# GadGadGad/Convolutional-KAN-for-Image-Classification

Hardware: AMD Instinct MI355X
Metric: images/sec fwd+bwd KAN-VGG11 3x32x32 bs=256/GPU (higher is better)
Workload: dtype f32

## Files before the change

### convolutional-kan-for-image-classification_amd/_lib.py

```python
from __future__ import annotations

import ctypes as C
import os
from typing import Optional

_HERE = os.path.dirname(os.path.abspath(__file__))
LIB_PATH = os.environ.get("KANCONV_LIB") or os.path.join(_HERE, "libkanconv.so")

KAN_MAX_PLANES = 16
KAN_MAX_TABLE = 32
KAN_FP_WORDS = 192
BASIS_BSPLINE, BASIS_RBF, BASIS_CHEBY, BASIS_POLY, BASIS_FOURIER, BASIS_RELU, BASIS_GRAM = 0, 1, 2, 3, 4, 5, 6
ACT_NONE, ACT_IDENTITY, ACT_GELU, ACT_SILU, ACT_RELU, ACT_TANH, ACT_SIGMOID, ACT_GELU_TANH = -1, 0, 1, 2, 3, 4, 5, 6
ORDER_QUAD_FWD, ORDER_ROWBLK8_FWD, ORDER_QUAD_BWD_DATA, ORDER_FWD_WEIGHT_SIDE = 1, 2, 4, 8


class KanGeom(C.Structure):
    _fields_ = [(n, C.c_int) for n in ("B", "C", "H", "W", "O", "Ho", "Wo", "kh", "kw", "sh", "sw", "ph", "pw", "dh", "dw", "groups")] + \
               [("x_bstride", C.c_longlong), ("y_bstride", C.c_longlong)]


class KanBasis(C.Structure):
    _fields_ = [("kind", C.c_int), ("n_basis", C.c_int), ("order", C.c_int), ("act", C.c_int),
                ("p0", C.c_float), ("p1", C.c_float), ("table", C.c_float * KAN_MAX_TABLE), ("chan_table", C.c_void_p)]


class KanPlan(C.Structure):
    _fields_ = [(n, C.c_int) for n in ("P", "K", "IPC", "KC", "Kpad", "Opad", "fwd_splits", "bwd_data_splits", "bwd_weight_splits",
                                          "fwd_target", "bwd_data_target", "bwd_weight_target", "x_pm_wanted", "dz_pm_wanted", "bwd_weight_expanded", "row_blocks", "e_pm_wanted", "fwd_expanded", "fwd_halo", "bwd_weight_halo",
                                          "fwd_band", "bwd_weight_band")] + \
               [(n, C.c_longlong) for n in ("packed_weight_bytes", "bwd_data_weight_bytes", "fwd_slab_elems", "bwd_data_slab_elems",
                                            "bwd_weight_slab_elems", "e_pm_elems")]


class KanNormRoute(C.Structure):
    _fields_ = [(n, C.c_int) for n in ("kernel", "G", "EPL", "PPI", "NT", "pool", "lds", "held", "blocks", "strided")]

# ... 127 lines not shown
```

### convolutional-kan-for-image-classification_amd/csrc/kan_internal.h

```cpp
#pragma once
#include <type_traits>
#include "kanconv.h"

int kan_fail_msg(const char* fmt, const char* a);
int kan_raise_lds_limit(const void* kernel, int bytes);

enum : int {
    FAST_GENERIC = 0,
    FAST_BSPLINE_SILU = 1,
    FAST_BSPLINE_GELU = 2,
    FAST_RBF8 = 3,
    FAST_CHEBY5 = 4,
    FAST_CHEBY4 = 5,
    FAST_POLY4 = 6,
    FAST_POLY3 = 7,
    FAST_RBF5 = 8,
    FAST_RELU8 = 9,
    FAST_GRAM4 = 10,
    FAST_POLY1 = 11,
    FAST_LAST = 11
};
enum : unsigned {
    ON_TAP_MAJOR = 1u << 0,
    ON_BIG_TILES = 1u << 1,
// ... 84 lines not shown
int kan_band_bwd_weight_launch(const float* dz, const float* x, const float* xn, float* dwp, const KanGeom* g, const KanBasis* b,
                               const KanBandCfg* cfg, int splits, long long slab_elems, void* stream);
int kan_band_fwd_launch(const float* x, const float* xn, const float* wp, float* z, const KanGeom* g, const KanBasis* b,
                        const KanBandCfg* cfg, int splits, long long slab_elems, void* stream);

constexpr int DW_T = 9;
constexpr int DW_MAX_TP = 96;

enum class Route { TAP_MAJOR, DW, BAND, HALO, EXPANDED };

struct FwdCfg { int TO, TP, tiles_o, tiles_p, chunks, splits, slots; };
struct BdCfg { int CH, tiles_c, tiles_p, n_ob, Opad32, chunks, splits; };
struct BwCfg { int TR, TO, tiles_r, tiles_o, chunks, splits, slots; };
struct BwHaloCfg { int R, nimg, spb, n_bands, tiles_r, tiles_o, splits, bands_per_split; };

struct ConvPlan {
    KanPlan pub;
    int fast;
    Route fwd, bwd_data, bwd_weight;
    bool pm_fwd, pm_bwd_data, pm_bwd_weight;
    bool rowblk_bwd_data;
    bool quad_fwd;
    bool quad_bd;
    bool rowblk8_fwd;
    bool fwd_wq;
    bool pmdma_xcd, pm_lpt, pm_xcd;
    FwdCfg fc;
    BdCfg bd;
    BwCfg bw;
    BwHaloCfg bwh;
    KanBandCfg band;
};
int plan_conv(const KanGeom* g, const KanBasis* b, ConvPlan* cp);

int live_taps_out(const KanGeom* g, int hw);
int live_taps_in(const KanGeom* g, int hw);
int live_positions_for_tap(const KanGeom* g, int tap);
int balance_tiles(const int* weight, int n, unsigned short* idx);
```

### convolutional-kan-for-image-classification_amd/csrc/kan_plan.hip

```cpp
#include <hip/hip_runtime.h>
#include <cstdio>
#include <cstdlib>
#include <cstring>
#include "kanconv.h"
#include "kan_device.h"
#include "kan_common.h"
#include "kan_internal.h"

namespace {

int fail(const char* msg) { return kan_fail_msg("%s", msg); }

int check(const KanGeom* g, const KanBasis* b) {
    if (!g || !b) return fail("null geometry/basis");
    if (g->groups < 0 || g->groups > 65535) return fail("groups out of range");
    if (g->B <= 0 || g->C <= 0 || g->O <= 0 || g->H <= 0 || g->W <= 0 || g->Ho <= 0 || g->Wo <= 0) return fail("non-positive dimension");
    if (g->kh <= 0 || g->kw <= 0 || g->sh <= 0 || g->sw <= 0 || g->dh <= 0 || g->dw <= 0 || g->ph < 0 || g->pw < 0) return fail("bad conv parameters");
    if (g->kh > 255 || g->kw > 255 || g->C > 65535) return fail("kernel size / channel count out of supported range");
    if ((g->H + 2 * g->ph - g->dh * (g->kh - 1) - 1) / g->sh + 1 != g->Ho || (g->W + 2 * g->pw - g->dw * (g->kw - 1) - 1) / g->sw + 1 != g->Wo)
        return fail("Ho/Wo inconsistent with H/W, kernel, stride, padding, dilation");
    if ((long long)g->B * g->Ho * g->Wo >= (1ll << 31) || (long long)g->B * g->H * g->W >= (1ll << 31)) return fail("pixel count exceeds int32");
    if ((long long)g->B * g->x_bstride * 4 >= (1ll << 31) || (long long)g->B * g->y_bstride * 4 >= (1ll << 31))
        return fail("activation tensors must be smaller than 2 GiB (32-bit buffer offsets)");
    if (g->x_bstride < (long long)ngroups(g) * g->C * g->H * g->W || g->y_bstride < (long long)ngroups(g) * g->O * g->Ho * g->Wo)
// ... 318 lines not shown
    pl->Opad = round_up(g->O, 64);
    pl->packed_weight_bytes = (long long)G * pl->Kpad * pl->Opad * 4;
    c.bd = bd_cfg(g, *pl);
    pl->bwd_data_weight_bytes = (long long)G * T * c.bd.Opad32 * c.bd.tiles_c * 128 * 4;
    pl->fwd_slab_elems = (long long)g->B * g->y_bstride;
    pl->bwd_data_slab_elems = (long long)g->B * g->x_bstride;
    pl->bwd_weight_slab_elems = (long long)G * pl->K * pl->Opad;
    const bool big = big_tiles(f, *pl);
    c.fc = fwd_cfg(g, *pl, big, c.pm_fwd, halo);
    c.bw = bw_cfg(g, *pl, big, c.pm_bwd_weight);
    if (halo_bw) c.bwh = bw_halo_cfg(g, *pl);
    pl->fwd_splits = band ? c.band.fwd_splits : c.fc.splits;
    pl->bwd_data_splits = c.bd.splits;
    pl->bwd_weight_splits = halo_bw ? c.bwh.splits : c.bw.splits;
    if (band_bw) {
        pl->bwd_weight_splits = c.band.bw_splits;
        pl->bwd_weight_slab_elems = (long long)G * pl->Kpad * pl->Opad;
    }
    pl->fwd_target = pl->bwd_data_target = pl->bwd_weight_target = 0;
    const bool rowblk_fwd = halo && g->H == 4 && g->W == 4 && c.fc.TO == 256;
    c.quad_fwd = rowblk_fwd && g->B % 32 == 0 && !tuning_off("KAN_QUAD_FWD");
    c.quad_bd = c.rowblk_bwd_data && g->B % 32 == 0 && !tuning_off("KAN_QUAD_BD");
    c.rowblk8_fwd = halo && g->H == 8 && g->W == 8 && c.fc.TO == 256 && g->B % 4 == 0 && !tuning_off("KAN_ROWBLK8_FWD");
    c.fwd_wq = c.fwd == Route::EXPANDED && g->H == 2 && g->W == 2 && g->Ho == 2 && g->Wo == 2 && g->kh == 3 && g->kw == 3 && g->sh == 1 && g->sw == 1 &&
               g->ph == 1 && g->pw == 1 && g->dh == 1 && g->dw == 1 && pl->P == 9 && pl->KC == 18 && g->y_bstride % 4 == 0 && !tuning_off("KAN_PMDMA_FWD_WQ");
    if (dw) {
        pl->fwd_splits = pl->bwd_data_splits = 1;
        pl->bwd_weight_splits = dw_weight_chunks(g);
        pl->bwd_data_weight_bytes = pl->packed_weight_bytes;
        c.pm_fwd = c.pm_bwd_data = c.pm_bwd_weight = false;
    }
    if (c.pm_fwd) {
        LiveClass cls[16]; const int plane = g->Ho * g->Wo;
        const long long tiles_per_pos = (long long)ceil_div(g->B, c.fc.TP) * c.fc.tiles_o * G;
        for (int hw = 0; hw < plane; ++hw) cls[hw] = LiveClass{tiles_per_pos, live_taps_out(g, hw) * ceil_div(g->C, pl->IPC)};
        pl->fwd_target = pick_target_steps(cls, plane, 8, 4.0 * g->B * g->O * g->Ho * g->Wo * G, &pl->fwd_splits, c.fc.slots);
    }
    if (c.pm_bwd_weight) {
        LiveClass cw[32];
        const long long tiles_per_tap = (long long)ceil_div((long long)g->C * pl->P, c.bw.TR) * c.bw.tiles_o * G;
        for (int tap = 0; tap < T; ++tap) cw[tap] = LiveClass{tiles_per_tap, live_positions_for_tap(g, tap) * ceil_div(g->B, 16)};
        pl->bwd_weight_target = pick_target_steps(cw, T, 16, 4.0 * pl->K * pl->Opad * G, &pl->bwd_weight_splits, c.bw.slots);
    }
    if (c.pm_bwd_data) {
        LiveClass cls[16]; const int plane = g->H * g->W;
        const long long tiles_per_pos = (long long)ceil_div(g->B, 128) * c.bd.tiles_c * G;
// ... 17 lines not shown
```

### convolutional-kan-for-image-classification_amd/csrc/kanconv.hip

```cpp
#include <hip/hip_runtime.h>
#include <cstdio>
#include <cstdlib>
#include <cstring>
#include <cmath>
#include <cstdint>
#include <mutex>
#include <type_traits>
#include <vector>
#include "kanconv.h"
#include "kan_device.h"

#include "kan_common.h"
#include "kan_internal.h"

namespace {


thread_local char g_err[512] = "";
int fail(const char* fmt, const char* a = "") {
    snprintf(g_err, sizeof(g_err), fmt, a);
    return -1;
}
}
int kan_fail_msg(const char* fmt, const char* a) { return fail(fmt, a); }
// ... 741 lines not shown
    do {                                                                                                                           \
        float fa_[2][2], fb_[2][2];                                                                                                \
        LDS_READ4(fa_[0][0], fa_[0][1], fb_[0][0], fb_[0][1], addrA, addrB, 0, 32 * 4, 0, 512 * 4);                                \
        _Pragma("unroll") for (int kk = 0; kk < (NK); ++kk) {                                                                       \
            const int c_ = kk & 1, n_ = c_ ^ 1;                                                                                    \
            if (kk + 1 < (NK)) {                                                                                                   \
                LDS_READ4(fa_[n_][0], fa_[n_][1], fb_[n_][0], fb_[n_][1], addrA, addrB, (2 * (kk + 1)) * (LDA) * 4,                \
                          (2 * (kk + 1)) * (LDA) * 4 + 128, (2 * (kk + 1)) * 32 * 4, (2 * (kk + 1)) * 32 * 4 + 512 * 4);           \
                LDS_WAIT4(fa_[c_][0], fa_[c_][1], fb_[c_][0], fb_[c_][1], 4);                                                      \
            } else {                                                                                                               \
                LDS_WAIT4(fa_[c_][0], fa_[c_][1], fb_[c_][0], fb_[c_][1], 0);                                                      \
            }                                                                                                                      \
            if (l0) {                                                                                                              \
                acc[0][0] = MFMA32(fa_[c_][0], fb_[c_][0], acc[0][0]);                                                             \
                acc[1][0] = MFMA32(fa_[c_][1], fb_[c_][0], acc[1][0]);                                                             \
            }                                                                                                                      \
            if (l1) {                                                                                                              \
                acc[0][1] = MFMA32(fa_[c_][0], fb_[c_][1], acc[0][1]);                                                             \
                acc[1][1] = MFMA32(fa_[c_][1], fb_[c_][1], acc[1][1]);                                                             \
            }                                                                                                                      \
        }                                                                                                                          \
    } while (0)

template <int KIND, int FAST, int RB = 0>
__global__ __launch_bounds__(256, 4) void k_conv_bwd_data(
    const float* __restrict__ dz, const float* __restrict__ x, const float* __restrict__ xn, const float* __restrict__ wd,
    float* __restrict__ dx, float* __restrict__ dxn, DevGeom g, DevBasis bs, int CH, int n_ct, int n_ob, int Opad16,
    int n_chunks, int chunks_per_split, long long slab_elems, unsigned dz_bytes, TilePerm perm, float* __restrict__ dpar) {
    constexpr int TP = 128, KD = 16, NT = 256;
    __shared__ __attribute__((aligned(16))) float smem[2 * 2 * KD * 128];
    __shared__ float sTab[KAN_MAX_TABLE];

    const int tid = threadIdx.x, lane = tid & 63;
    const int wave = __builtin_amdgcn_readfirstlane(tid >> 6);
    const int w_r = wave >> 1, w_p = wave & 1;
    const int HoWo = g.Ho * g.Wo, HW = g.H * g.W, P = bs.P;
    const int Min = g.B * HW;
    const BlockId blk = xcd_block_order(false);
    const int grp = blk.y / n_ct;
    const int px_tile0 = (perm.n ? (int)perm.idx[blk.x] : blk.x) * TP, ct = blk.y - grp * n_ct;
    const int ncol = n_ct * 128;
    const int pxl = (wave & 1) * 64 + lane, ol0 = wave >> 1;
    const bool idle_rows = (ct * 2 + w_r) * CH >= g.C;
    {
        const size_t xo = (size_t)grp * g.C * HW;
        x += xo; xn += xo; dx += xo; if (dxn) dxn += xo;
        dz += (size_t)grp * g.O * HoWo * ((g.pix_major || RB == 2) ? g.B : 1);
        wd += (size_t)grp * (g.kh * g.kw) * Opad16 * ncol;
    }

    if (tid < KAN_MAX_TABLE) sTab[tid] = bs.tab[tid];
    const int q_qh = (blk.x >> 1) & 1, q_qw = blk.x & 1, q_b0 = (blk.x >> 2) * 32;
    auto q_pos = [&](int bk) { return ((bk == 0 || bk == 2) ? 3 * q_qh : 1 + q_qh) * 4 + ((bk == 0 || bk == 3) ? 3 * q_qw : 1 + q_qw); };
    auto q_mask = [&](int hw) {
        unsigned m = 0;
        for (int tap = 0; tap < 9; ++tap) {
            const int r = tap / 3, t = tap - r * 3;
            m |= (((unsigned)((hw >> 2) + 1 - r) < 4u && (unsigned)((hw & 3) + 1 - t) < 4u) ? 1u : 0u) << tap;
        }
        return m;
    };
    const int my_px = RB == 2 ? (q_b0 + (pxl & 31)) * 16 + q_pos(pxl >> 5)
                              : px_tile0 + (RB == 1 ? ((pxl >> 2) & 7) * 16 + (pxl >> 5) * 4 + (pxl & 3) : pxl);
    const bool pv = my_px < Min;
    int pb, ph_, pw_;
    {
        int hw;
        if (g.pix_major) { hw = my_px / g.B; pb = my_px - hw * g.B; }
        else { pb = my_px / HW; hw = my_px - pb * HW; }
        ph_ = hw / g.W; pw_ = hw - ph_ * g.W;
// ... 89 lines not shown
    const unsigned q_live0 = q_mask(q_pos(2 * w_p)), q_live1 = q_mask(q_pos(2 * w_p + 1));
    const unsigned q_voff = (unsigned)((lane >> 3) * 16 * g.B + (lane & 7) * 4) * 4u;
    int pend_tap = 0;
    auto issue_q = [&](int ch, int buf) {
        const int tap = ch / n_ob, o0 = (ch - tap * n_ob) * KD;
        pend_tap = tap;
        float* dW = smem + buf * (2 * KD * 128);
        float* dG = dW + KD * 128 + wv * 512;
        if ((cp_live >> tap) & 1u) {
            const int r = tap / 3, t = tap - r * 3;
            const unsigned so = (unsigned)((o0 * 16 + cp_hw + (1 - r) * 4 + (1 - t)) * g.B + q_b0) * 4u;
            __builtin_amdgcn_raw_ptr_buffer_load_lds(dz_rs, (__attribute__((address_space(3))) void*)dG, 16, (int)q_voff, (int)so, 0, 0);
            __builtin_amdgcn_raw_ptr_buffer_load_lds(dz_rs, (__attribute__((address_space(3))) void*)(dG + 256), 16, (int)q_voff,
                                                     (int)(so + (unsigned)(8 * 16 * g.B) * 4u), 0, 0);
        }
        const char* wsrc = (const char*)(wd + ((size_t)tap * Opad16 + o0) * ncol + ct * 128);
#pragma unroll
        for (int j = 0; j < 2; ++j) {
            const int blk2 = j * 4 + wv;
            glds16((const float*)(wsrc + (size_t)blk2 * 2 * ncol * 4 + wlane), dW + blk2 * 256);
        }
    };

    f32x16 acc[2][2];
#pragma unroll
    for (int a = 0; a < 2; ++a)
#pragma unroll
        for (int b = 0; b < 2; ++b)
#pragma unroll
            for (int r = 0; r < 16; ++r) acc[a][b][r] = 0.f;

    int ch0 = blk.z * chunks_per_split;
    int ch1 = min(n_chunks, ch0 + chunks_per_split);
    unsigned tapmask = 0xffffffffu;
    if (g.pix_major) {
        tapmask = 0;
        const int T = g.kh * g.kw;
        const int hwA = px_tile0 / g.B, hwB = min(px_tile0 + TP - 1, Min - 1) / g.B;
        for (int hw = hwA; hw <= hwB; ++hw)
            for (int tap = 0; tap < T; ++tap) tapmask |= (tap_alive_in(g, hw, tap) ? 1u : 0u) << tap;
        auto seg = [&](int tap) { return tap * n_ob; };
        const int L = live_step_count(tapmask, T, n_chunks, seg);
        const int S = min((int)gridDim.z, max(1, (L + chunks_per_split - 1) / chunks_per_split));
        if (blk.z >= S) { ch0 = ch1 = n_chunks; }
        else {
            ch0 = blk.z == 0 ? 0 : live_step_pos(tapmask, T, n_chunks, (int)((long long)L * blk.z / S), seg);
            ch1 = blk.z == S - 1 ? n_chunks : live_step_pos(tapmask, T, n_chunks, (int)((long long)L * (blk.z + 1) / S), seg);
        }
    }
    auto next_live = [&](int ch) -> int {
        if (!g.pix_major) return ch;
        while (ch < ch1) {
            const int tap = ch / n_ob;
            if ((tapmask >> tap) & 1u) return ch;
            ch = (tap + 1) * n_ob;
        }
        return ch1;
    };
    int ch = next_live(ch0);
    if (ch < ch1) { if (RB == 2) issue_q(ch, 0); else if (RB) issue_rb(ch, 0); else issue(ch, 0); }
    const int ar = w_r * 64 + (lane & 31), bp = w_p * 64 + (lane & 31), kh2 = lane >> 5;
    for (int cur = 0; ch < ch1; cur ^= 1) {
        asm volatile("s_waitcnt vmcnt(0)" ::: "memory");
        __syncthreads();
        const bool mixed_now = pend_mixed;
        const int tap_now = pend_tap;
        ch = next_live(ch + 1);
        if (ch < ch1) { if (RB == 2) issue_q(ch, cur ^ 1); else if (RB) issue_rb(ch, cur ^ 1); else issue(ch, cur ^ 1); }
        const float* cW = smem + cur * (2 * KD * 128);
        const float* cG = cW + KD * 128;
        const unsigned aw = lds_addr(cW + kh2 * 128 + ar), ag = lds_addr(cG + kh2 * TP + bp);
        if (RB == 2) {
            const unsigned agq = lds_addr(cG + (2 * w_p) * 512 + kh2 * 32 + (lane & 31));
            const bool l0 = ((q_live0 >> tap_now) & 1u) != 0, l1 = ((q_live1 >> tap_now) & 1u) != 0;
            if (!idle_rows) KAN_MFMA_STEP_QUAD(KD / 2, aw, 128, agq, l0, l1);
        } else if (RB) {
            const bool l0b = !(mixed_now && w_p == 0), l1a = !(mixed_now && w_p == 1);
            if (!idle_rows) KAN_MFMA_STEP_LIVE(KD / 2, aw, 128, ag, TP, true, l0b, l1a, true);
        } else if (!idle_rows) KAN_MFMA_STEP(KD / 2, aw, 128, ag, TP);
    }

    const bool same_in = (x == xn);
    const bool split_out = (dxn != nullptr);
    float* dxs = dx + (size_t)blk.z * slab_elems;
    float* dxns = split_out ? dxn + (size_t)blk.z * slab_elems : nullptr;
#define KAN_G_TO_LDS(half)                                                                                                 \
    __syncthreads();                                                                                                       \
    if (w_r == (half)) {                                                                                                   \
        _Pragma("unroll") for (int mi = 0; mi < 2; ++mi)                                                                   \
            _Pragma("unroll") for (int ni = 0; ni < 2; ++ni)                                                               \
                _Pragma("unroll") for (int r = 0; r < 16; ++r)                                                             \
                    smem[(mi * 32 + mfma_row(r, lane)) * TP + w_p * 64 + ni * 32 + (lane & 31)] = acc[mi][ni][r];          \
    }                                                                                                                      \
    __syncthreads();
    if constexpr (FAST != 0) {
        constexpr FastSpec S = fast_spec(FAST);
        constexpr int FP = S.planes, FCH = 64 / FP, NIT = (FCH + 1) / 2, NPF = S.xn_bwd ? 1 : 2;
        float xv[NPF][NIT], nv[NIT]; unsigned ok = 0;
#define KAN_FETCH(half, slot)                                                                                              \
        _Pragma("unroll") for (int it = 0; it < NIT; ++it) {                                                                   \
            const int cl = ol0 + 2 * it, c = (ct * 2 + (half)) * FCH + cl;                                                     \
            const bool v = cl < FCH && c < g.C && pv;                                                                          \
            const size_t idx = (size_t)pb * g.xbs + (size_t)c * HW + (size_t)(ph_ * g.W + pw_);                                \
            xv[slot][it] = v ? x[idx] : 0.f;                                                                                   \
            if constexpr (S.xn_bwd) nv[it] = v ? xn[idx] : 0.f;                                                                \
            ok |= (v ? 1u : 0u) << ((slot) * NIT + it);                                                                        \
        }
        if constexpr (!S.xn_bwd) {
#pragma unroll
            for (int half = 0; half < 2; ++half) KAN_FETCH(half, half)
        }
#pragma unroll 1
        for (int half = 0; half < 2; ++half) {
            if constexpr (S.xn_bwd) { ok = 0; KAN_FETCH(half, 0) }
            KAN_G_TO_LDS(half)
#pragma unroll
            for (int it = 0; it < NIT; ++it) {
                if (!((ok >> ((S.xn_bwd ? 0 : half) * NIT + it)) & 1u)) continue;
                const int cl = ol0 + 2 * it, c = (ct * 2 + half) * FCH + cl;
                const float xa = (S.xn_bwd || half == 0) ? xv[0][it] : xv[NPF - 1][it];
// ... 1721 lines not shown
        const int bx = c.tiles_c * 4, by = c.Opad32 / 32 * G;
        const long long nt = (long long)bx * by;
        const long long capd = fp ? 128 : 1024;
        dim3 gd((unsigned)(nt < capd ? nt : capd), 1, T);
        hipLaunchKernelGGL(k_pack_bwd_data, gd, dim3(256), 0, st, (const float*)wp, wd, q, c.CH, c.tiles_c, c.Opad32, wp_gs, bx, by, fp, fp_cur);
    }
    return launch_ok("pack");
}

int kan_pack_weights(const float* w_base, const float* w_basis, float* wp, float* wd, const KanGeom* g, const KanBasis* b, void* stream) {
    return pack_weights_impl(w_base, w_basis, wp, wd, g, b, nullptr, 0, stream);
}

int kan_pack_weights_iod(const float* coeffs, float* wp, float* wd, const KanGeom* g, const KanBasis* b, void* stream) {
    if (int rc = iod_scope(g, b)) return rc;
    return pack_weights_impl(nullptr, coeffs, wp, wd, g, b, nullptr, 0, stream, true);
}

int kan_tile_orders(const KanGeom* g, const KanBasis* b) {
    ConvPlan cp;
    if (plan_conv(g, b, &cp)) return 0;
    const bool halo = cp.fwd == Route::HALO;
    return (halo && cp.quad_fwd ? KAN_ORDER_QUAD_FWD : 0) | (halo && cp.rowblk8_fwd ? KAN_ORDER_ROWBLK8_FWD : 0) | (cp.quad_bd ? KAN_ORDER_QUAD_BWD_DATA : 0) |
           (cp.fwd_wq ? KAN_ORDER_FWD_WEIGHT_SIDE : 0);
}

int kan_pack_cacheable(const KanGeom* g, const KanBasis* b) {
    ConvPlan cp;
    if (plan_conv(g, b, &cp)) return 0;
    if ((long long)g->O * g->C * (b->n_basis + 1) * g->kh * g->kw >= (1ll << 31)) return 0;
    return (!pack_needs_clear(g, cp.pub) && cp.fwd != Route::DW && ngroups(g) == 1) ? 1 : 0;
}

int kan_pack_weights_cached(const float* w_base, const float* w_basis, float* wp, float* wd, const KanGeom* g, const KanBasis* b,
                            unsigned long long* ring, int cur, int force, int sample_stride, void* stream) {
    static_assert(KAN_FP_WORDS == 3 * FP_LANES, "ring size");
    if (!ring || cur < 0 || cur > 2 || sample_stride < 1) return fail("bad fingerprint ring arguments");
    if (!kan_pack_cacheable(g, b)) return fail("cached packing is not offered for this geometry (kan_pack_cacheable)");
    const int hb = b->act != KAN_ACT_NONE;
    if ((hb && !w_base) || !w_basis) return fail("null weight pointer");
    if (((size_t)w_basis & 15) || (hb && ((size_t)w_base & 15))) return fail("cached packing needs 16-byte aligned weight tensors");
    const int T = g->kh * g->kw;
    const long long na = hb ? (long long)g->O * g->C * T : 0, nbs = (long long)g->O * g->C * b->n_basis * T;
    const long long groups4 = ((na + 3) / 4 + (nbs + 3) / 4 + sample_stride - 1) / sample_stride;
    long long blocks = (groups4 + 256 * 8 - 1) / (256 * 8); if (blocks > 4096) blocks = 4096; if (blocks < 1) blocks = 1;
    hipLaunchKernelGGL(k_fingerprint, dim3((unsigned)blocks), dim3(256), 0, (hipStream_t)stream, hb ? w_base : w_basis, (unsigned)na, w_basis,
                       (unsigned)nbs, (unsigned)sample_stride, ring, cur);
// ... 166 lines not shown
        DevGeom dgd = dev_geom(g); DevBasis dbd = dev_basis(b);
        dim3 grid(ceil_div((long long)g->B * g->H * g->W, 256), ngroups(g));
        dispatch_kind(b->kind, [&](auto kind) {
            hipLaunchKernelGGL((k_dw_bwd_data<decltype(kind)::value>), grid, dim3(256), 0, st, dz, x, xn, wd, dx, dxn, dgd, dbd, pl.Opad, pl.IPC, pl.KC, pl.Kpad);
        });
        return launch_ok("dw_bwd_data");
    }
    const BdCfg& c = cp.bd;
    DevGeom dg = dev_geom(g);
    dg.pix_major = (dz_pm && cp.pm_bwd_data) ? 1 : 0;
    if (dg.pix_major) dz = dz_pm;
    DevBasis db = dev_basis(b);
    if ((long long)c.tiles_c * ngroups(g) > 65535) return fail("groups * channel tiles exceed the grid limit");
    dim3 grid(c.tiles_p, c.tiles_c * ngroups(g), pl.bwd_data_splits);
    const int cps = dg.pix_major ? pl.bwd_data_target : ceil_div(c.chunks, pl.bwd_data_splits);
    TilePerm perm; perm.n = 0;
    if (dg.pix_major) perm = tile_perm(c.tiles_p, [&](int t) {
        const int hw = (int)(((long long)t * 128) / g->B);
        return ceil_div(live_taps_in(g, hw < g->H * g->W ? hw : 0) * c.n_ob, cps > 0 ? cps : 1);
    });
    const int fast = (fast_spec(cp.fast).xn_bwd ? (x != xn && dxn) : (x == xn && !dxn)) ? cp.fast : FAST_GENERIC;
    const bool rb = !dg.pix_major && cp.rowblk_bwd_data;
    const bool quad = rb && cp.quad_bd && dz_pm && x == xn && !dxn;
    const unsigned dz_bytes = (unsigned)((long long)g->B * g->y_bstride * 4);
    auto launch = [&](auto kind, auto fast, auto rbv) {
        hipLaunchKernelGGL((k_conv_bwd_data<decltype(kind)::value, decltype(fast)::value, decltype(rbv)::value>), grid, dim3(256), 0, st,
                           decltype(rbv)::value == 2 ? dz_pm : dz, x, xn, wd,
                           dx, dxn, dg, db, c.CH, c.tiles_c, c.n_ob, c.Opad32, c.chunks, cps, pl.bwd_data_slab_elems, dz_bytes, perm, dpar);
    };
    const bool launched = dispatch_fast<ON_TAP_MAJOR>(fast, [&](auto fv) {
        constexpr int F = decltype(fv)::value;
        if constexpr (fast_has(F, ON_ROWBLK_BWD_DATA)) {
            if (quad) return launch(IC<fast_kind(F)>{}, fv, IC<2>{});
            if (rb) return launch(IC<fast_kind(F)>{}, fv, IC<1>{});
        }
        launch(IC<fast_kind(F)>{}, fv, IC<0>{});
    });
    if (!launched) dispatch_kind(b->kind, [&](auto kind) { launch(kind, IC<FAST_GENERIC>{}, IC<0>{}); });
    return launch_ok("conv_bwd_data");
}

int kan_conv_bwd_weight(const float* dz, const float* x, const float* xn, float* dwp, const KanGeom* g, const KanBasis* b,
                        const float* x_pm, const float* dz_pm, void* stream) {
    ConvPlan cp;
    if (int rc = plan_conv(g, b, &cp)) return rc;
    const KanPlan& pl = cp.pub;
    if (!dz || !x || !xn || !dwp) return fail("null tensor pointer");
    if ((b->kind == KAN_BASIS_RELU || b->kind == KAN_BASIS_GRAM) && !b->chan_table) return fail("ReLU / Gram bases need their device parameter table (chan_table)");
    hipStream_t st = (hipStream_t)stream;
    if (cp.bwd_weight == Route::DW) {
        DevGeom dgd = dev_geom(g); DevBasis dbd = dev_basis(b);
        dim3 grid(pl.bwd_weight_splits, ngroups(g));
        dispatch_kind(b->kind, [&](auto kind) {
            hipLaunchKernelGGL((k_dw_bwd_weight<decltype(kind)::value>), grid, dim3(256), 0, st, dz, x, xn, dwp, dgd, dbd, pl.K, pl.Opad, pl.bwd_weight_slab_elems);
        });
// ... 381 lines not shown
```

### convolutional-kan-for-image-classification_amd/ops.py

```python
from __future__ import annotations

import contextlib
import ctypes as C
import os
import weakref
from collections import OrderedDict
from dataclasses import dataclass, replace
from functools import lru_cache, partial, wraps
from typing import List, NamedTuple, Optional, Sequence, Tuple

import torch
from torch.autograd.function import once_differentiable

from . import _lib as L


@dataclass(frozen=True)
class ConvSpec:
    kind: int
    n_basis: int
    order: int
    act: int
    p0: float
    p1: float
# ... 157 lines not shown
        for wo in range(Wo):
            for r in range(kh):
                for t in range(kw):
                    hi, wi = ho * sh - ph + r * dh, wo * sw - pw + t * dw
                    live += 0 <= hi < H and 0 <= wi < W
    return live / float(Ho * Wo * kh * kw)


_ROW_BLOCK_BIT = {"fwd": 1, "bwd_data": 2, "bwd_weight": 0}


def _quadrant_order(geom, plan, which: str) -> bool:
    return which == "fwd" and bool(plan.row_blocks & 1) and geom.B % 32 == 0


def _quadrant_bwd_data(geom, plan, have_dz_pm: bool) -> bool:
    return bool(have_dz_pm) and bool(plan.row_blocks & 2) and bool(getattr(plan, "tile_orders", 0) & L.ORDER_QUAD_BWD_DATA)


def _row_blocks8_forward(geom, plan) -> bool:
    return geom.H == 8 and geom.W == 8 and bool(getattr(plan, "tile_orders", 0) & L.ORDER_ROWBLK8_FWD)


def _executed_flops(geom, plan, which: str, have_dz_pm: bool = False) -> float:
    target = {"fwd": plan.fwd_target, "bwd_data": plan.bwd_data_target, "bwd_weight": plan.bwd_weight_target}[which]
    dense = _conv_flops(geom, plan)
    g = geom
    if target <= 0:
        if _quadrant_order(geom, plan, which) or (which == "bwd_data" and _quadrant_bwd_data(geom, plan, have_dz_pm)):
            return dense * _live_fraction(which, g.H, g.W, g.Ho, g.Wo, g.kh, g.kw, g.sh, g.sw, g.ph, g.pw, g.dh, g.dw)
        if plan.row_blocks & _ROW_BLOCK_BIT[which]:
            return dense * (5.0 / 6.0)
        if which == "fwd" and _row_blocks8_forward(geom, plan):
            return dense * (11.0 / 12.0)
        return dense
    return dense * _live_fraction(which, g.H, g.W, g.Ho, g.Wo, g.kh, g.kw, g.sh, g.sw, g.ph, g.pw, g.dh, g.dw)


def _layer_tag(geom) -> str:
    return f"{geom.C * max(1, geom.groups)}->{geom.O * max(1, geom.groups)}@{geom.H}x{geom.W} k{geom.kh}x{geom.kw}"


def _sample(which: str, geom, plan, pm: bool, two: bool = False, expanded: bool = False):
    tile = "128" if plan.Opad % 128 == 0 else "64"
    if which == "bwd_data":
        name = "k_conv_bwd_data"
    elif expanded:
        name = f"k_conv_{which}_pmdma/o{tile}"
    elif plan.fwd_band if which == "fwd" else plan.bwd_weight_band:
        name = f"k_band_{which}/o" + ("128" if plan.Opad % 128 == 0 else "192" if plan.Opad == 192 else "64")
    else:
        halo = plan.fwd_halo if which == "fwd" else (plan.bwd_weight_halo and not two)
        name = f"k_conv_{which}{'_halo' if halo else ''}/o{tile}"
    skips = expanded or pm or bool(plan.row_blocks & _ROW_BLOCK_BIT[which]) or (which == "fwd" and _row_blocks8_forward(geom, plan))
    dense = _conv_flops(geom, plan)
    return name, dense, _executed_flops(geom, plan, which, pm) if skips else dense, _layer_tag(geom)

# ... 379 lines not shown
    ent.used = True
    return t


def _conv_backward(spec: ConvSpec, x, xn, packed, dz, need_x: bool, need_xn: bool, need_w: bool, phases=None, mode: int = 0, wids=None, dparams=None, wcd=None, dw_split: bool = False):
    lib = L.load()
    B, Ct, H, W = x.shape
    G = spec.groups
    Cg = Ct // G
    Ot = dz.shape[1]
    Og = Ot // G
    geom, basis, plan = _plan_cached(*_plan_key(spec, x.shape, Og))
    basis = _with_table(_with_phases(basis, phases, mode), spec, x.device)
    kh, kw = spec.kernel
    st = _stream(x)
    xs = xn if xn is not None else x
    wd, x_pm = packed
    dw_base: List[Optional[torch.Tensor]] = [None] * G
    dw_basis: List[Optional[torch.Tensor]] = [None] * G
    split_w = need_w and dw_split
    split_x = need_x and wcd is not None
    exact_w = need_w and not split_w
    exact_x = (need_x or need_xn) and not split_x
    dz_pm = _position_major(dz, 0, Ot) if (plan.dz_pm_wanted and xn is None and (exact_w or exact_x)) else None
    if split_w:
        sb, ss = (_sink_for(wids[0], (Og, Cg, kh, kw), x.device), _sink_for(wids[1], (Og, Cg * spec.n_basis, kh, kw), x.device)) if wids else (None, None)
        dwb = sb if sb is not None else torch.empty((Og, Cg, kh, kw), device=x.device, dtype=torch.float32)
        dws = ss if ss is not None else torch.empty((Og, Cg * spec.n_basis, kh, kw), device=x.device, dtype=torch.float32)
        kan_conv_bwd_weight_split(spec, x, dz, out=(dwb, dws))
        dw_base, dw_basis = list(dwb.unsqueeze(0).unbind(0)), list(dws.unsqueeze(0).unbind(0))
    elif exact_w:
        dwp = torch.empty(plan.bwd_weight_splits * plan.bwd_weight_slab_elems, device=x.device, dtype=torch.float32)
        if plan.bwd_weight_expanded and xn is None and dz_pm is not None:
            e_pm = x_pm if (plan.fwd_expanded and not plan.x_pm_wanted and x_pm is not None and mode == 0) else _expand_pm(x, geom, basis, plan, st)
            _launch(_sample("bwd_weight", geom, plan, True, expanded=True), x,
                    lambda: lib.kan_conv_bwd_weight_expanded(_ptr(dz_pm), _ptr(e_pm), _ptr(dwp), C.byref(geom), C.byref(basis), st))
        else:
            _launch(_sample("bwd_weight", geom, plan, x_pm is not None and dz_pm is not None, xn is not None), x,
                    lambda: lib.kan_conv_bwd_weight(_ptr(dz), _ptr(x), _ptr(xs), _ptr(dwp), C.byref(geom), C.byref(basis), _ptr(x_pm),
                                                    _ptr(dz_pm), st))
        if spec.w_layout == W_IOD:
            dco = torch.empty((Cg, Og, spec.n_basis), device=x.device, dtype=torch.float32)
            L.check(lib.kan_unpack_wgrad_iod(_ptr(dwp), _ptr(dco), C.byref(geom), C.byref(basis), st), "kan_unpack_wgrad_iod")
            dw_basis = [dco]
        else:
            sb = _sink_for(wids[0], (Og, Cg, kh, kw), x.device) if (wids and G == 1 and spec.has_base) else None
            ss = _sink_for(wids[1], (Og, Cg * spec.n_basis, kh, kw), x.device) if (wids and G == 1) else None
# ... 612 lines not shown
```

### include/kanconv.h

```cpp
#ifndef KANCONV_H
#define KANCONV_H

#ifdef __cplusplus
extern "C" {
#endif

#define KAN_MAX_PLANES 16
#define KAN_MAX_TABLE  32
#define KAN_FP_WORDS   192

enum { KAN_BASIS_BSPLINE = 0, KAN_BASIS_RBF = 1, KAN_BASIS_CHEBY = 2, KAN_BASIS_POLY = 3, KAN_BASIS_FOURIER = 4, KAN_BASIS_RELU = 5, KAN_BASIS_GRAM = 6 };
enum { KAN_ACT_NONE = -1, KAN_ACT_IDENTITY = 0, KAN_ACT_GELU = 1, KAN_ACT_SILU = 2, KAN_ACT_RELU = 3,
       KAN_ACT_TANH = 4, KAN_ACT_SIGMOID = 5, KAN_ACT_GELU_TANH = 6 };

typedef struct KanGeom {
    int B, C, H, W;
    int O, Ho, Wo;
    int kh, kw, sh, sw, ph, pw, dh, dw;
    int groups;
    long long x_bstride;
    long long y_bstride;
} KanGeom;

#define KAN_ORDER_PACK(mode, first) ((int)(mode) | ((int)(first) << 8))
// ... 18 lines not shown
    int x_pm_wanted, dz_pm_wanted;
    int bwd_weight_expanded;
    int row_blocks;
    int e_pm_wanted, fwd_expanded;
    int fwd_halo, bwd_weight_halo;
    int fwd_band, bwd_weight_band;
    long long packed_weight_bytes;
    long long bwd_data_weight_bytes;
    long long fwd_slab_elems;
    long long bwd_data_slab_elems;
    long long bwd_weight_slab_elems;
    long long e_pm_elems;
} KanPlan;

const char* kan_version(void);
const char* kan_last_error(void);

int kan_plan(const KanGeom* geom, const KanBasis* basis, KanPlan* plan);

#define KAN_ORDER_QUAD_FWD 1
#define KAN_ORDER_ROWBLK8_FWD 2
#define KAN_ORDER_QUAD_BWD_DATA 4
#define KAN_ORDER_FWD_WEIGHT_SIDE 8
int kan_tile_orders(const KanGeom* geom, const KanBasis* basis);

int kan_pack_weights(const float* w_base, const float* w_basis, float* wp, float* wd,
                     const KanGeom* geom, const KanBasis* basis, void* stream);

int kan_pack_weights_iod(const float* coeffs, float* wp, float* wd, const KanGeom* geom, const KanBasis* basis, void* stream);

int kan_pack_cacheable(const KanGeom* geom, const KanBasis* basis);
int kan_pack_weights_cached(const float* w_base, const float* w_basis, float* wp, float* wd,
                            const KanGeom* geom, const KanBasis* basis, unsigned long long* ring, int cur, int force,
                            int sample_stride, void* stream);

int kan_conv_fwd(const float* x, const float* xn, const float* wp, float* z,
                 const KanGeom* geom, const KanBasis* basis, const float* x_pm, void* stream);

int kan_position_major(const float* src, float* dst, int B, int Cn, int HW, long long bstride, void* stream);

int kan_conv_bwd_data(const float* dz, const float* x, const float* xn, const float* wd,
                      float* dx, float* dxn,
                      const KanGeom* geom, const KanBasis* basis, const float* dz_pm, void* stream);

int kan_conv_bwd_data_params(const float* dz, const float* x, const float* xn, const float* wd, float* dx, float* dxn, float* dparams,
                             const KanGeom* geom, const KanBasis* basis, const float* dz_pm, void* stream);
// ... 169 lines not shown
```

Measured before the change: 18110.

## Add position-major 8x8 backward-data tile route with border tap skipping

Adds an RB==3 variant of the backward-data kernel for 8x8 3x3 stride-1 layers. Each block covers a 32-image by 4-column strip of one row, loading position-major dz directly into LDS through buffer loads. The variant skips dead taps at row borders and dead MFMA sub-tiles at column borders, and uses a permuted tile order plus a per-live-step split. It also adds a vectorized float4 epilogue. Dz is now converted to position-major for these layers even when it was not otherwise wanted, which adds an extra transpose pass.

```diff
diff --git a/convolutional-kan-for-image-classification_amd/_lib.py b/convolutional-kan-for-image-classification_amd/_lib.py
--- a/convolutional-kan-for-image-classification_amd/_lib.py
+++ b/convolutional-kan-for-image-classification_amd/_lib.py
@@ -12,7 +12,7 @@
 KAN_FP_WORDS = 192
 BASIS_BSPLINE, BASIS_RBF, BASIS_CHEBY, BASIS_POLY, BASIS_FOURIER, BASIS_RELU, BASIS_GRAM = 0, 1, 2, 3, 4, 5, 6
 ACT_NONE, ACT_IDENTITY, ACT_GELU, ACT_SILU, ACT_RELU, ACT_TANH, ACT_SIGMOID, ACT_GELU_TANH = -1, 0, 1, 2, 3, 4, 5, 6
-ORDER_QUAD_FWD, ORDER_ROWBLK8_FWD, ORDER_QUAD_BWD_DATA, ORDER_FWD_WEIGHT_SIDE = 1, 2, 4, 8
+ORDER_QUAD_FWD, ORDER_ROWBLK8_FWD, ORDER_QUAD_BWD_DATA, ORDER_FWD_WEIGHT_SIDE, ORDER_POS8_BWD_DATA = 1, 2, 4, 8, 16
 
 
 class KanGeom(C.Structure):
diff --git a/convolutional-kan-for-image-classification_amd/csrc/kan_internal.h b/convolutional-kan-for-image-classification_amd/csrc/kan_internal.h
--- a/convolutional-kan-for-image-classification_amd/csrc/kan_internal.h
+++ b/convolutional-kan-for-image-classification_amd/csrc/kan_internal.h
@@ -130,6 +130,7 @@
     bool rowblk_bwd_data;
     bool quad_fwd;
     bool quad_bd;
+    bool pos8_bd;
     bool rowblk8_fwd;
     bool fwd_wq;
     bool pmdma_xcd, pm_lpt, pm_xcd;
diff --git a/convolutional-kan-for-image-classification_amd/csrc/kan_plan.hip b/convolutional-kan-for-image-classification_amd/csrc/kan_plan.hip
--- a/convolutional-kan-for-image-classification_amd/csrc/kan_plan.hip
+++ b/convolutional-kan-for-image-classification_amd/csrc/kan_plan.hip
@@ -364,6 +364,9 @@
     c.quad_fwd = rowblk_fwd && g->B % 32 == 0 && !tuning_off("KAN_QUAD_FWD");
     c.quad_bd = c.rowblk_bwd_data && g->B % 32 == 0 && !tuning_off("KAN_QUAD_BD");
     c.rowblk8_fwd = halo && g->H == 8 && g->W == 8 && c.fc.TO == 256 && g->B % 4 == 0 && !tuning_off("KAN_ROWBLK8_FWD");
+    c.pos8_bd = !tuning_off("KAN_POS8_BD") && fast_has(f, ON_ROWBLK_BWD_DATA) && !c.pm_bwd_data && !dw && g->H == 8 && g->W == 8 && g->Ho == 8 && g->Wo == 8 &&
+                g->kh == 3 && g->kw == 3 && g->sh == 1 && g->sw == 1 && g->ph == 1 && g->pw == 1 && g->dh == 1 && g->dw == 1 && g->B % 32 == 0 &&
+                g->O % 16 == 0 && g->x_bstride % 4 == 0 && (long long)g->O * 64 * g->B * 4 < (1ll << 31);
     c.fwd_wq = c.fwd == Route::EXPANDED && g->H == 2 && g->W == 2 && g->Ho == 2 && g->Wo == 2 && g->kh == 3 && g->kw == 3 && g->sh == 1 && g->sw == 1 &&
                g->ph == 1 && g->pw == 1 && g->dh == 1 && g->dw == 1 && pl->P == 9 && pl->KC == 18 && g->y_bstride % 4 == 0 && !tuning_off("KAN_PMDMA_FWD_WQ");
     if (dw) {
diff --git a/convolutional-kan-for-image-classification_amd/csrc/kanconv.hip b/convolutional-kan-for-image-classification_amd/csrc/kanconv.hip
--- a/convolutional-kan-for-image-classification_amd/csrc/kanconv.hip
+++ b/convolutional-kan-for-image-classification_amd/csrc/kanconv.hip
@@ -787,6 +787,32 @@
         }                                                                                                                          \
     } while (0)
 
+#define LDS_READ5(ra, r0, r1, r2, r3, addrA, addrB, oA, oB)                                                                              \
+    asm volatile("ds_read_b32 %0, %5 offset:%7\n\tds_read_b32 %1, %6 offset:%8\n\tds_read_b32 %2, %6 offset:%9\n\t"                    \
+                 "ds_read_b32 %3, %6 offset:%10\n\tds_read_b32 %4, %6 offset:%11"                                                        \
+                 : "=&v"(ra), "=&v"(r0), "=&v"(r1), "=&v"(r2), "=&v"(r3)                                                                \
+                 : "v"(addrA), "v"(addrB), "n"(oA), "n"(oB), "n"((oB) + 512 * 4), "n"((oB) + 1024 * 4), "n"((oB) + 1536 * 4) : "memory")
+#define LDS_WAIT5(ra, r0, r1, r2, r3, N) asm volatile("s_waitcnt lgkmcnt(" #N ")" : "+v"(ra), "+v"(r0), "+v"(r1), "+v"(r2), "+v"(r3) :: "memory")
+#define KAN_MFMA_STEP_POS8(NK, addrA, LDA, addrB, l0, l3)                                                                           \
+    do {                                                                                                                           \
+        float fa_[2], fb_[2][4];                                                                                                   \
+        LDS_READ5(fa_[0], fb_[0][0], fb_[0][1], fb_[0][2], fb_[0][3], addrA, addrB, 0, 0);                                         \
+        _Pragma("unroll") for (int kk = 0; kk < (NK); ++kk) {                                                                       \
+            const int c_ = kk & 1, n_ = c_ ^ 1;                                                                                    \
+            if (kk + 1 < (NK)) {                                                                                                   \
+                LDS_READ5(fa_[n_], fb_[n_][0], fb_[n_][1], fb_[n_][2], fb_[n_][3], addrA, addrB, (2 * (kk + 1)) * (LDA) * 4,       \
+                          (2 * (kk + 1)) * 32 * 4);                                                                                \
+                LDS_WAIT5(fa_[c_], fb_[c_][0], fb_[c_][1], fb_[c_][2], fb_[c_][3], 5);                                             \
+            } else {                                                                                                               \
+                LDS_WAIT5(fa_[c_], fb_[c_][0], fb_[c_][1], fb_[c_][2], fb_[c_][3], 0);                                             \
+            }                                                                                                                      \
+            if (l0) acc[0][0] = MFMA32(fa_[c_], fb_[c_][0], acc[0][0]);                                                            \
+            acc[0][1] = MFMA32(fa_[c_], fb_[c_][1], acc[0][1]);                                                                    \
+            acc[1][0] = MFMA32(fa_[c_], fb_[c_][2], acc[1][0]);                                                                    \
+            if (l3) acc[1][1] = MFMA32(fa_[c_], fb_[c_][3], acc[1][1]);                                                            \
+        }                                                                                                                          \
+    } while (0)
+
 template <int KIND, int FAST, int RB = 0>
 __global__ __launch_bounds__(256, 4) void k_conv_bwd_data(
     const float* __restrict__ dz, const float* __restrict__ x, const float* __restrict__ xn, const float* __restrict__ wd,
@@ -806,11 +832,18 @@
     const int px_tile0 = (perm.n ? (int)perm.idx[blk.x] : blk.x) * TP, ct = blk.y - grp * n_ct;
     const int ncol = n_ct * 128;
     const int pxl = (wave & 1) * 64 + lane, ol0 = wave >> 1;
-    const bool idle_rows = (ct * 2 + w_r) * CH >= g.C;
+    const bool idle_rows = RB == 3 ? (ct * 2 + w_r) * CH * P + w_p * 32 >= g.C * P || w_p * 32 >= CH * P : (ct * 2 + w_r) * CH >= g.C;
+    int p8_tile = blk.x;
+    if (RB == 3) {
+        const int ng = (int)gridDim.x >> 4, nmid = 12 * ng;
+        if (blk.x < nmid) { const int k = blk.x / ng; p8_tile = (blk.x - k * ng) * 16 + 2 + k; }
+        else { const int y = blk.x - nmid, cls = y >= 2 * ng ? 1 : 0, y2 = y - cls * 2 * ng, k = y2 / ng; p8_tile = (y2 - k * ng) * 16 + cls * 14 + k; }
+    }
+    const int p8_b0 = (p8_tile >> 4) * 32, p8_h = (p8_tile >> 1) & 7, p8_w0 = (p8_tile & 1) * 4;
     {
         const size_t xo = (size_t)grp * g.C * HW;
         x += xo; xn += xo; dx += xo; if (dxn) dxn += xo;
-        dz += (size_t)grp * g.O * HoWo * ((g.pix_major || RB == 2) ? g.B : 1);
+        dz += (size_t)grp * g.O * HoWo * ((g.pix_major || RB >= 2) ? g.B : 1);
         wd += (size_t)grp * (g.kh * g.kw) * Opad16 * ncol;
     }
 
@@ -946,6 +979,28 @@
         }
     };
 
+    const int p8_col = p8_w0 + wv;
+    const unsigned p8_voff = (unsigned)((lane >> 3) * 64 * g.B + (lane & 7) * 4) * 4u;
+    auto issue_p8 = [&](int ch, int buf) {
+        const int tap = ch / n_ob, o0 = (ch - tap * n_ob) * KD;
+        pend_tap = tap;
+        float* dW = smem + buf * (2 * KD * 128);
+        float* dG = dW + KD * 128 + wv * 512;
+        const int r = tap / 3, t = tap - r * 3;
+        if ((unsigned)(p8_col + 1 - t) < 8u) {
+            const unsigned so = (unsigned)((o0 * 64 + (p8_h + 1 - r) * 8 + (p8_col + 1 - t)) * g.B + p8_b0) * 4u;
+            __builtin_amdgcn_raw_ptr_buffer_load_lds(dz_rs, (__attribute__((address_space(3))) void*)dG, 16, (int)p8_voff, (int)so, 0, 0);
+            __builtin_amdgcn_raw_ptr_buffer_load_lds(dz_rs, (__attribute__((address_space(3))) void*)(dG + 256), 16, (int)p8_voff,
+                                                     (int)(so + (unsigned)(8 * 64 * g.B) * 4u), 0, 0);
+        }
+        const char* wsrc = (const char*)(wd + ((size_t)tap * Opad16 + o0) * ncol + ct * 128);
+#pragma unroll
+        for (int j = 0; j < 2; ++j) {
+            const int blk2 = j * 4 + wv;
+            glds16((const float*)(wsrc + (size_t)blk2 * 2 * ncol * 4 + wlane), dW + blk2 * 256);
+        }
+    };
+
     f32x16 acc[2][2];
 #pragma unroll
     for (int a = 0; a < 2; ++a)
@@ -957,15 +1012,20 @@
     int ch0 = blk.z * chunks_per_split;
     int ch1 = min(n_chunks, ch0 + chunks_per_split);
     unsigned tapmask = 0xffffffffu;
-    if (g.pix_major) {
+    const bool skip_taps = g.pix_major || RB == 3;
+    if (skip_taps) {
         tapmask = 0;
         const int T = g.kh * g.kw;
-        const int hwA = px_tile0 / g.B, hwB = min(px_tile0 + TP - 1, Min - 1) / g.B;
-        for (int hw = hwA; hw <= hwB; ++hw)
-            for (int tap = 0; tap < T; ++tap) tapmask |= (tap_alive_in(g, hw, tap) ? 1u : 0u) << tap;
+        if (RB == 3) {
+            for (int r = 0; r < 3; ++r) tapmask |= ((unsigned)(p8_h + 1 - r) < 8u ? 7u : 0u) << (3 * r);
+        } else {
+            const int hwA = px_tile0 / g.B, hwB = min(px_tile0 + TP - 1, Min - 1) / g.B;
+            for (int hw = hwA; hw <= hwB; ++hw)
+                for (int tap = 0; tap < T; ++tap) tapmask |= (tap_alive_in(g, hw, tap) ? 1u : 0u) << tap;
+        }
         auto seg = [&](int tap) { return tap * n_ob; };
         const int L = live_step_count(tapmask, T, n_chunks, seg);
-        const int S = min((int)gridDim.z, max(1, (L + chunks_per_split - 1) / chunks_per_split));
+        const int S = RB == 3 ? min((int)gridDim.z, max(1, L)) : min((int)gridDim.z, max(1, (L + chunks_per_split - 1) / chunks_per_split));
         if (blk.z >= S) { ch0 = ch1 = n_chunks; }
         else {
             ch0 = blk.z == 0 ? 0 : live_step_pos(tapmask, T, n_chunks, (int)((long long)L * blk.z / S), seg);
@@ -973,7 +1033,7 @@
         }
     }
     auto next_live = [&](int ch) -> int {
-        if (!g.pix_major) return ch;
+        if (!skip_taps) return ch;
         while (ch < ch1) {
             const int tap = ch / n_ob;
             if ((tapmask >> tap) & 1u) return ch;
@@ -981,8 +1041,11 @@
         }
         return ch1;
     };
+    auto issue_step = [&](int ch, int buf) {
+        if (RB == 3) issue_p8(ch, buf); else if (RB == 2) issue_q(ch, buf); else if (RB) issue_rb(ch, buf); else issue(ch, buf);
+    };
     int ch = next_live(ch0);
-    if (ch < ch1) { if (RB == 2) issue_q(ch, 0); else if (RB) issue_rb(ch, 0); else issue(ch, 0); }
+    if (ch < ch1) issue_step(ch, 0);
     const int ar = w_r * 64 + (lane & 31), bp = w_p * 64 + (lane & 31), kh2 = lane >> 5;
     for (int cur = 0; ch < ch1; cur ^= 1) {
         asm volatile("s_waitcnt vmcnt(0)" ::: "memory");
@@ -990,11 +1053,16 @@
         const bool mixed_now = pend_mixed;
         const int tap_now = pend_tap;
         ch = next_live(ch + 1);
-        if (ch < ch1) { if (RB == 2) issue_q(ch, cur ^ 1); else if (RB) issue_rb(ch, cur ^ 1); else issue(ch, cur ^ 1); }
+        if (ch < ch1) issue_step(ch, cur ^ 1);
         const float* cW = smem + cur * (2 * KD * 128);
         const float* cG = cW + KD * 128;
         const unsigned aw = lds_addr(cW + kh2 * 128 + ar), ag = lds_addr(cG + kh2 * TP + bp);
-        if (RB == 2) {
+        if (RB == 3) {
+            const unsigned aw8 = lds_addr(cW + kh2 * 128 + wave * 32 + (lane & 31)), ag8 = lds_addr(cG + kh2 * 32 + (lane & 31));
+            const int t_now = tap_now % 3;
+            const bool l0 = !(p8_w0 == 0 && t_now == 2), l3 = !(p8_w0 == 4 && t_now == 0);
+            if (!idle_rows) KAN_MFMA_STEP_POS8(KD / 2, aw8, 128, ag8, l0, l3);
+        } else if (RB == 2) {
             const unsigned agq = lds_addr(cG + (2 * w_p) * 512 + kh2 * 32 + (lane & 31));
             const bool l0 = ((q_live0 >> tap_now) & 1u) != 0, l1 = ((q_live1 >> tap_now) & 1u) != 0;
             if (!idle_rows) KAN_MFMA_STEP_QUAD(KD / 2, aw, 128, agq, l0, l1);
@@ -1020,6 +1088,46 @@
     if constexpr (FAST != 0) {
         constexpr FastSpec S = fast_spec(FAST);
         constexpr int FP = S.planes, FCH = 64 / FP, NIT = (FCH + 1) / 2, NPF = S.xn_bwd ? 1 : 2;
+        if constexpr (RB == 3) {
+            constexpr int NQ = (FCH + 7) / 8;
+            const int img = tid & 31, cl0 = tid >> 5;
+            const size_t pix = (size_t)(p8_b0 + img) * g.xbs + (size_t)(p8_h * 8 + p8_w0);
+            float4 xq[2][NQ]; unsigned okq = 0;
+#pragma unroll
+            for (int half = 0; half < 2; ++half)
+#pragma unroll
+                for (int it = 0; it < NQ; ++it) {
+                    const int cl = cl0 + 8 * it, c = (ct * 2 + half) * FCH + cl;
+                    const bool v = cl < FCH && c < g.C;
+                    xq[half][it] = v ? *reinterpret_cast<const float4*>(x + pix + (size_t)c * HW) : make_float4(0.f, 0.f, 0.f, 0.f);
+                    okq |= (v ? 1u : 0u) << (half * NQ + it);
+                }
+#pragma unroll
+            for (int half = 0; half < 2; ++half) {
+                __syncthreads();
+                if (w_r == half) {
+#pragma unroll
+                    for (int j = 0; j < 4; ++j)
+#pragma unroll
+                        for (int r = 0; r < 16; ++r) smem[(w_p * 32 + mfma_row(r, lane)) * TP + j * 32 + (lane & 31)] = acc[j >> 1][j & 1][r];
+                }
+                __syncthreads();
+#pragma unroll
+                for (int it = 0; it < NQ; ++it) {
+                    if (!((okq >> (half * NQ + it)) & 1u)) continue;
+                    const int cl = cl0 + 8 * it, c = (ct * 2 + half) * FCH + cl;
+                    const float4 xa = xq[half][it];
+                    const float* Gc = smem + (cl * FP) * TP + img;
+                    float4 d;
+                    d.x = stage_unit_grad<KIND, FAST>(bs, sTab, xa.x, xa.x, Gc, TP).dx;
+                    d.y = stage_unit_grad<KIND, FAST>(bs, sTab, xa.y, xa.y, Gc + 32, TP).dx;
+                    d.z = stage_unit_grad<KIND, FAST>(bs, sTab, xa.z, xa.z, Gc + 64, TP).dx;
+                    d.w = stage_unit_grad<KIND, FAST>(bs, sTab, xa.w, xa.w, Gc + 96, TP).dx;
+                    *reinterpret_cast<float4*>(dxs + pix + (size_t)c * HW) = d;
+                }
+            }
+            return;
+        }
         float xv[NPF][NIT], nv[NIT]; unsigned ok = 0;
 #define KAN_FETCH(half, slot)                                                                                              \
         _Pragma("unroll") for (int it = 0; it < NIT; ++it) {                                                                   \
@@ -2787,7 +2895,7 @@
     if (plan_conv(g, b, &cp)) return 0;
     const bool halo = cp.fwd == Route::HALO;
     return (halo && cp.quad_fwd ? KAN_ORDER_QUAD_FWD : 0) | (halo && cp.rowblk8_fwd ? KAN_ORDER_ROWBLK8_FWD : 0) | (cp.quad_bd ? KAN_ORDER_QUAD_BWD_DATA : 0) |
-           (cp.fwd_wq ? KAN_ORDER_FWD_WEIGHT_SIDE : 0);
+           (cp.fwd_wq ? KAN_ORDER_FWD_WEIGHT_SIDE : 0) | (cp.pos8_bd ? KAN_ORDER_POS8_BWD_DATA : 0);
 }
 
 int kan_pack_cacheable(const KanGeom* g, const KanBasis* b) {
@@ -3000,15 +3108,17 @@
     const int fast = (fast_spec(cp.fast).xn_bwd ? (x != xn && dxn) : (x == xn && !dxn)) ? cp.fast : FAST_GENERIC;
     const bool rb = !dg.pix_major && cp.rowblk_bwd_data;
     const bool quad = rb && cp.quad_bd && dz_pm && x == xn && !dxn;
-    const unsigned dz_bytes = (unsigned)((long long)g->B * g->y_bstride * 4);
+    const bool pos8 = cp.pos8_bd && !dg.pix_major && dz_pm && x == xn && !dxn && !dpar && ((uintptr_t)x | (uintptr_t)dx) % 16 == 0;
+    const unsigned dz_bytes = pos8 ? (unsigned)((long long)g->O * g->Ho * g->Wo * g->B * 4) : (unsigned)((long long)g->B * g->y_bstride * 4);
     auto launch = [&](auto kind, auto fast, auto rbv) {
         hipLaunchKernelGGL((k_conv_bwd_data<decltype(kind)::value, decltype(fast)::value, decltype(rbv)::value>), grid, dim3(256), 0, st,
-                           decltype(rbv)::value == 2 ? dz_pm : dz, x, xn, wd,
+                           decltype(rbv)::value >= 2 ? dz_pm : dz, x, xn, wd,
                            dx, dxn, dg, db, c.CH, c.tiles_c, c.n_ob, c.Opad32, c.chunks, cps, pl.bwd_data_slab_elems, dz_bytes, perm, dpar);
     };
     const bool launched = dispatch_fast<ON_TAP_MAJOR>(fast, [&](auto fv) {
         constexpr int F = decltype(fv)::value;
         if constexpr (fast_has(F, ON_ROWBLK_BWD_DATA)) {
+            if (pos8) return launch(IC<fast_kind(F)>{}, fv, IC<3>{});
             if (quad) return launch(IC<fast_kind(F)>{}, fv, IC<2>{});
             if (rb) return launch(IC<fast_kind(F)>{}, fv, IC<1>{});
         }
diff --git a/convolutional-kan-for-image-classification_amd/ops.py b/convolutional-kan-for-image-classification_amd/ops.py
--- a/convolutional-kan-for-image-classification_amd/ops.py
+++ b/convolutional-kan-for-image-classification_amd/ops.py
@@ -203,6 +203,10 @@
     return geom.H == 8 and geom.W == 8 and bool(getattr(plan, "tile_orders", 0) & L.ORDER_ROWBLK8_FWD)
 
 
+def _pos8_bwd_data(geom, plan) -> bool:
+    return bool(getattr(plan, "tile_orders", 0) & L.ORDER_POS8_BWD_DATA)
+
+
 def _executed_flops(geom, plan, which: str, have_dz_pm: bool = False) -> float:
     target = {"fwd": plan.fwd_target, "bwd_data": plan.bwd_data_target, "bwd_weight": plan.bwd_weight_target}[which]
     dense = _conv_flops(geom, plan)
@@ -214,6 +218,8 @@
             return dense * (5.0 / 6.0)
         if which == "fwd" and _row_blocks8_forward(geom, plan):
             return dense * (11.0 / 12.0)
+        if which == "bwd_data" and have_dz_pm and _pos8_bwd_data(geom, plan):
+            return dense * (484.0 / 576.0)
         return dense
     return dense * _live_fraction(which, g.H, g.W, g.Ho, g.Wo, g.kh, g.kw, g.sh, g.sw, g.ph, g.pw, g.dh, g.dw)
 
@@ -639,7 +645,7 @@
     split_x = need_x and wcd is not None
     exact_w = need_w and not split_w
     exact_x = (need_x or need_xn) and not split_x
-    dz_pm = _position_major(dz, 0, Ot) if (plan.dz_pm_wanted and xn is None and (exact_w or exact_x)) else None
+    dz_pm = _position_major(dz, 0, Ot) if (xn is None and ((plan.dz_pm_wanted and (exact_w or exact_x)) or (exact_x and _pos8_bwd_data(geom, plan)))) else None
     if split_w:
         sb, ss = (_sink_for(wids[0], (Og, Cg, kh, kw), x.device), _sink_for(wids[1], (Og, Cg * spec.n_basis, kh, kw), x.device)) if wids else (None, None)
         dwb = sb if sb is not None else torch.empty((Og, Cg, kh, kw), device=x.device, dtype=torch.float32)
diff --git a/include/kanconv.h b/include/kanconv.h
--- a/include/kanconv.h
+++ b/include/kanconv.h
@@ -64,6 +64,7 @@
 #define KAN_ORDER_ROWBLK8_FWD 2
 #define KAN_ORDER_QUAD_BWD_DATA 4
 #define KAN_ORDER_FWD_WEIGHT_SIDE 8
+#define KAN_ORDER_POS8_BWD_DATA 16
 int kan_tile_orders(const KanGeom* geom, const KanBasis* basis);
 
 int kan_pack_weights(const float* w_base, const float* w_basis, float* wp, float* wd,
```

Measured after the change: 18300 (median of 6 runs). 1.1% higher.
